# davidea97/Fisher-Nerf-customized

Hardware: AMD Instinct MI355X
Metric: candidate-views/sec (higher is better)
Workload: dtype f32

## Files before the change

### fisher-nerf-customized_amd/csrc/fisher_rast.hip

```cpp
#include <hip/hip_runtime.h>
#include <hip/hip_fp16.h>
#include <stdint.h>
#include <stdio.h>
#include <stdlib.h>
#include <string.h>
#include "fr_math.h"
#include "../../include/fisher_rast.h"
#include "fr_internal.h"

#define FR_THREADS 256
#define FR_G_MAX 32
#define FR_MAX_LDS_TILES 4096
#define FR_PART_MIN_DEFAULT 2048
#define FR_SORT_SMALL_KEYS 2048
#define FR_SORT_MID_KEYS 4096
#define FR_SORT_BIG_KEYS 16384
#define FR_VC_MAX 16
#define FR_BATCH 256
#define FR_BWD_BATCH 128

#include <vector>
#include <utility>
static thread_local char g_err[512] = "";
#if defined(FR_ABLATE) || defined(FR_LOOPSTATS)
#ifndef FR_AB
#define FR_AB
#endif
#endif
#ifdef FR_AB
#define FR_AB_ONLY(x) x
static int fr_debug_mode();
static int fr_env_int(const char* name) { const char* e = getenv(name); return e ? atoi(e) : 0; }
#else
#define FR_AB_ONLY(x)
static constexpr int fr_debug_mode() { return 0; }
#endif
static bool g_prof_on = false;
static std::vector<std::pair<hipEvent_t, hipEvent_t>> g_prof_events;
int fr_fail(int code, const char* msg)
{
	snprintf(g_err, sizeof(g_err), "%s", msg);
	return code;
}
int fr_check_launch(const char* what)
{
	hipError_t e = hipGetLastError();
	if (e != hipSuccess)
	{
		snprintf(g_err, sizeof(g_err), "%s: %s", what, hipGetErrorString(e));
		return FR_ELAUNCH;
	}
	return FR_OK;
}

struct FrSplat { float x, y, cx, cy, cz, o, depth; uint32_t ext; };

struct FrVisEntry { uint32_t idx, depth_bits, xy0, xy1; };

struct FrParams {
	int P, V, W, H;
	uint32_t gx, gy;
	int T;
	int G;
	float tanfovx, tanfovy, focal_x, focal_y, mod;
	int D, M;
	const float* bg; const float* view; const float* proj; const float* campos;
	const float* w2c;
	const float* means3D; const float* colors; const float* shs; const float* opac;
	const float* scales; const float* rots;
	const float* cov3D;
	float* cov3D_out;
	int* radii;
	FrSplat* splat;
	float* rgb;
	uint8_t* clamped;
	uint32_t* tile_cnt; uint32_t* tile_off; uint32_t* tile_fill;
	uint64_t* keys; long long key_capacity;
	uint32_t* blk_base;
	uint32_t* big_list;
	uint32_t* view_work;
	uint32_t* view_perm;
	int* status;
	int* vis_count;
	int* num_rendered;
	struct FrVisEntry* vis_list;
	uint32_t* vis_n;
	int VC;
	uint32_t tile_cap;
	uint32_t small_max;
	const uint32_t* order;
	int legacy_sort;
	int prefiltered;
	int ablate;
};
#ifdef FR_ABLATE
#define FR_ABL(x) x
#else
#define FR_ABL(x)
#endif

__device__ __forceinline__ float wave_sum(float v)
{
#pragma unroll
	for (int o = 32; o > 0; o >>= 1) v += __shfl_xor(v, o, 64);
	return v;
}
__device__ __forceinline__ int wave_max_i(int v)
{
#pragma unroll
	for (int o = 32; o > 0; o >>= 1) { int t = __shfl_xor(v, o, 64); v = t > v ? t : v; }
	return v;
}

__device__ __forceinline__ bool fr_any(bool x) { return __builtin_amdgcn_ballot_w64(x) != 0ull; }
__device__ __forceinline__ bool fr_all(bool x) { return __builtin_amdgcn_ballot_w64(!x) == 0ull; }
__device__ __forceinline__ float fr_readlane_f(float x, int l) { return __int_as_float(__builtin_amdgcn_readlane(__float_as_int(x), l)); }
__device__ __forceinline__ float fr_bperm_f(float x, int l) { return __int_as_float(__builtin_amdgcn_ds_bpermute(l << 2, __float_as_int(x))); }

__device__ __forceinline__ float fr_exp_hw(float x) { return __builtin_amdgcn_exp2f(x * 1.44269504088896341f); }

__device__ __forceinline__ float fr_power_threshold(float opacity)
{
	return (opacity > 0.f) ? (-__logf(255.0f * opacity) - 0.01f) : INFINITY;
}

__device__ __forceinline__ uint32_t fr_alpha_extent(float cx, float cy, float cz, float opacity)
{
	const float thr = fr_power_threshold(opacity);
	float hx = INFINITY, hy = INFINITY;
	if (!(thr <= 0.f)) { hx = -1.f; hy = -1.f; }
	else
	{
		const float det = cx * cz - cy * cy;
		if (det > 0.f && cx > 0.f && cz > 0.f)
		{
			const float tau2 = -2.0f * thr;
			const float ex = sqrtf(tau2 * cz / det) * 1.01f + 0.01f;
			const float ey = sqrtf(tau2 * cx / det) * 1.01f + 0.01f;
			if (ex == ex && ey == ey) { hx = ex; hy = ey; }
		}
	}
	const __half2 h = __halves2half2(__float2half_ru(hx), __float2half_ru(hy));
	return *(const uint32_t*)&h;
}

__global__ __launch_bounds__(FR_THREADS) void k_cov3d(int P, const float* __restrict__ scales, float mod,
                                                      const float* __restrict__ rots, float* __restrict__ cov3D)
{
	int i = blockIdx.x * FR_THREADS + threadIdx.x;
	if (i >= P) return;
	fr_f3 s = { scales[3 * i], scales[3 * i + 1], scales[3 * i + 2] };
	fr_f4 q = { rots[4 * i], rots[4 * i + 1], rots[4 * i + 2], rots[4 * i + 3] };
	float c[6];
	fr_cov3d(s, mod, q, c);
#pragma unroll
	for (int k = 0; k < 6; k++) cov3D[6 * (size_t)i + k] = c[k];
}

__global__ __launch_bounds__(FR_THREADS) void k_mark_visible(int P, const float* __restrict__ means3D,
                                                             const float* __restrict__ view, uint8_t* __restrict__ present)
{
	int i = blockIdx.x * FR_THREADS + threadIdx.x;
	if (i >= P) return;
	float vm[16];
#pragma unroll
	for (int k = 0; k < 16; k++) vm[k] = view[k];
	fr_f3 p = { means3D[3 * i], means3D[3 * i + 1], means3D[3 * i + 2] };
	fr_f3 pv = fr_xform4x3(p, vm);
	present[i] = (pv.z <= 0.001f) ? 0 : 1;
}

__global__ __launch_bounds__(FR_THREADS) void k_preprocess(FrParams p)
{
	extern __shared__ uint32_t fr_dyn_lds[];
// ... 1021 lines not shown
		{
			const int v = v0 + vv;
			uint32_t* cnt = p.tile_cnt + (size_t)v * p.T;
			const uint32_t* h = hist + (size_t)vv * p.T;
			for (int t = tid; t < p.T; t += FR_THREADS)
			{
				const uint32_t c = h[t];
				if (c) p.blk_base[((size_t)v * nblk + blockIdx.x) * p.T + t] = atomicAdd(&cnt[t], c);
			}
		}
	}
	if (tid < nv)
	{
		const int v = v0 + tid;
		p.vis_n[(size_t)v * nblk + blockIdx.x] = s_n[tid];
		if (p.vis_count && s_n[tid]) atomicAdd(&p.vis_count[v], (int)s_n[tid]);
		if (p.num_rendered && s_ref[tid]) atomicAdd(&p.num_rendered[v], (int)s_ref[tid]);
	}
}
__global__ __launch_bounds__(FR_THREADS) void k_scatter_vis(FrParams p)
{
	extern __shared__ uint32_t fr_dyn_lds[];
	uint32_t* s_cnt = fr_dyn_lds;
	uint32_t* s_base = fr_dyn_lds + p.T;
	if (p.status[1]) return;
	const int tid = threadIdx.x;
	const int v = blockIdx.y;
	const uint32_t nblk = gridDim.x;
	const uint32_t n = p.vis_n[(size_t)v * nblk + blockIdx.x];
	if (n == 0) return;
	const uint32_t* off = p.tile_off + (size_t)v * p.T;
	const uint32_t* bb = p.blk_base + ((size_t)v * nblk + blockIdx.x) * p.T;
	for (int t = tid; t < p.T; t += FR_THREADS) { s_cnt[t] = 0; s_base[t] = off[t] + bb[t]; }
	__syncthreads();
	const uint4* list = (const uint4*)(p.vis_list + ((size_t)v * nblk + blockIdx.x) * (size_t)(FR_THREADS * p.G));
	constexpr int NB = 4;
	for (uint32_t e0 = 0; e0 < n; e0 += NB * FR_THREADS)
	{
		uint4 en[NB];
#pragma unroll
		for (int b = 0; b < NB; b++)
		{
			const uint32_t e = e0 + b * FR_THREADS + tid;
			en[b] = e < n ? list[e] : make_uint4(0u, 0u, 0u, 0u);
		}
#pragma unroll
		for (int b = 0; b < NB; b++)
		{
			const uint64_t key = ((uint64_t)en[b].y << 32) | en[b].x;
			const uint32_t x0 = en[b].z & 0xffffu, y0 = en[b].z >> 16, x1 = en[b].w & 0xffffu, y1 = en[b].w >> 16;
			for (uint32_t y = y0; y < y1; y++)
				for (uint32_t x = x0; x < x1; x++)
				{
					const uint32_t t = y * p.gx + x;
					p.keys[s_base[t] + atomicAdd(&s_cnt[t], 1u)] = key;
				}
		}
	}
}

__device__ __forceinline__ void fr_tile_of_block(const FrParams& p, uint32_t& tile, int& v)
{
	const uint32_t L = blockIdx.x;
	if ((p.V & 7) == 0)
	{
		const uint32_t xcd = L & 7u, q = L >> 3;
		v = (int)((q / (uint32_t)p.T) * 8u + xcd);
		if (p.view_perm) v = (int)p.view_perm[v];
		tile = q % (uint32_t)p.T;
	}
	else
	{
		v = (int)(L / (uint32_t)p.T);
		tile = L % (uint32_t)p.T;
	}
}

__device__ __forceinline__ void fr_cx(uint64_t& lo, uint64_t& hi)
{
	const uint64_t a = lo, b = hi;
	const bool sw = a > b;
	lo = sw ? b : a; hi = sw ? a : b;
}
template <typename KeyPtr>
__device__ __forceinline__ uint64_t fr_ldk(KeyPtr keys, uint32_t i, uint32_t n) { return i < n ? keys[i] : ~0ull; }
template <typename KeyPtr>
__device__ __forceinline__ void fr_stk(KeyPtr keys, uint32_t i, uint32_t n, uint64_t v) { if (i < n) keys[i] = v; }

template <typename KeyPtr>
__device__ __forceinline__ void fr_bitonic(KeyPtr keys, uint32_t n, int tid, const uint32_t FR_NT = FR_THREADS)
{
	uint32_t n_pad = 1;
	while (n_pad < n) n_pad <<= 1;
	if (n_pad < 2) return;
	for (uint32_t t = tid; t < (n_pad >> 1); t += FR_NT)
	{
		uint64_t a = fr_ldk(keys, 2 * t, n), b = fr_ldk(keys, 2 * t + 1, n);
		fr_cx(a, b);
		fr_stk(keys, 2 * t, n, a); fr_stk(keys, 2 * t + 1, n, b);
	}
	__syncthreads();
	const uint32_t groups = n_pad >> 2;
	for (uint32_t k = 4, lk = 2; k <= n_pad; k <<= 1, lk++)
	{
		{
			const uint32_t q = k >> 2, qm = q - 1u;
			for (uint32_t g = tid; g < groups; g += FR_NT)
			{
				const uint32_t base = (g >> (lk - 2)) << lk, r = g & qm;
				const uint32_t ia = base + r, ib = ia + q, id = base + k - 1u - r, ic = id - q;
				uint64_t a = fr_ldk(keys, ia, n), b = fr_ldk(keys, ib, n), c = fr_ldk(keys, ic, n), d = fr_ldk(keys, id, n);
				fr_cx(a, d); fr_cx(b, c);
				fr_cx(a, b); fr_cx(c, d);
				fr_stk(keys, ia, n, a); fr_stk(keys, ib, n, b); fr_stk(keys, ic, n, c); fr_stk(keys, id, n, d);
			}
			__syncthreads();
		}
		uint32_t j = k >> 3, lj = lk - 3;
		for (; j >= 2; j >>= 2, lj -= 2)
		{
			const uint32_t h = j >> 1, lh = lj - 1, hm = h - 1u;
			for (uint32_t g = tid; g < groups; g += FR_NT)
			{
				const uint32_t i0 = ((g >> lh) << (lh + 2)) + (g & hm);
				const uint32_t i1 = i0 + h, i2 = i0 + j, i3 = i2 + h;
				uint64_t a = fr_ldk(keys, i0, n), b = fr_ldk(keys, i1, n), c = fr_ldk(keys, i2, n), d = fr_ldk(keys, i3, n);
				fr_cx(a, c); fr_cx(b, d);
				fr_cx(a, b); fr_cx(c, d);
				fr_stk(keys, i0, n, a); fr_stk(keys, i1, n, b); fr_stk(keys, i2, n, c); fr_stk(keys, i3, n, d);
			}
			__syncthreads();
		}
		if (j == 1)
		{
			for (uint32_t t = tid; t < (n_pad >> 1); t += FR_NT)
			{
				uint64_t a = fr_ldk(keys, 2 * t, n), b = fr_ldk(keys, 2 * t + 1, n);
				fr_cx(a, b);
				fr_stk(keys, 2 * t, n, a); fr_stk(keys, 2 * t + 1, n, b);
			}
			__syncthreads();
		}
	}
}

__device__ __forceinline__ uint64_t fr_shfl64(uint64_t v, int src_lane)
{
	const int lo = __builtin_amdgcn_ds_bpermute(src_lane << 2, (int)(uint32_t)v);
	const int hi = __builtin_amdgcn_ds_bpermute(src_lane << 2, (int)(uint32_t)(v >> 32));
	return ((uint64_t)(uint32_t)hi << 32) | (uint64_t)(uint32_t)lo;
}
__device__ __forceinline__ void fr_take(uint64_t& mine, uint64_t other, bool keepmin)
{
	const bool take = (other < mine) == keepmin;
	mine = take ? other : mine;
}
template <int CTRL>
__device__ __forceinline__ uint64_t fr_dpp64(uint64_t v)
{
	const int lo = __builtin_amdgcn_mov_dpp((int)(uint32_t)v, CTRL, 0xf, 0xf, false);
	const int hi = __builtin_amdgcn_mov_dpp((int)(uint32_t)(v >> 32), CTRL, 0xf, 0xf, false);
	return ((uint64_t)(uint32_t)hi << 32) | (uint64_t)(uint32_t)lo;
}
template <int ROWS>
__device__ __forceinline__ void fr_take_rows(uint64_t& key, bool keepmin)
{
	const uint32_t l = (uint32_t)key, h = (uint32_t)(key >> 32);
	uint64_t a, b;
	if constexpr (ROWS == 16)
	{
		const auto tl = __builtin_amdgcn_permlane16_swap(l, l, false, false);
		const auto th = __builtin_amdgcn_permlane16_swap(h, h, false, false);
		a = ((uint64_t)th[0] << 32) | tl[0]; b = ((uint64_t)th[1] << 32) | tl[1];
	}
	else
	{
		const auto tl = __builtin_amdgcn_permlane32_swap(l, l, false, false);
		const auto th = __builtin_amdgcn_permlane32_swap(h, h, false, false);
		a = ((uint64_t)th[0] << 32) | tl[0]; b = ((uint64_t)th[1] << 32) | tl[1];
	}
	key = ((b < a) == keepmin) ? b : a;
}

template <int K> struct FrLog2 { static constexpr int value = K == 1 ? 0 : K == 2 ? 1 : K == 4 ? 2 : K == 8 ? 3 : 4; };
template <int M>
__device__ __forceinline__ void fr_take_lane_xor(uint64_t& key, bool keepmin)
{
	if constexpr (M == 0) fr_take(key, fr_dpp64<0xB1>(key), keepmin);
	else if constexpr (M == 1) fr_take(key, fr_dpp64<0x4E>(key), keepmin);
	else if constexpr (M == 2) fr_take(key, fr_dpp64<0x141>(fr_dpp64<0x1B>(key)), keepmin);
	else if constexpr (M == 3) fr_take(key, fr_dpp64<0x128>(key), keepmin);
	else if constexpr (M == 4) fr_take_rows<16>(key, keepmin);
	else fr_take_rows<32>(key, keepmin);
}
template <int M>
__device__ __forceinline__ uint64_t fr_lane_mirror(uint64_t key, int lane)
{
	if constexpr (M == 1) return fr_dpp64<0xB1>(key);
	else if constexpr (M == 2) return fr_dpp64<0x1B>(key);
	else if constexpr (M == 3) return fr_dpp64<0x141>(key);
	else if constexpr (M == 4) return fr_dpp64<0x140>(key);
	else return fr_shfl64(key, lane ^ ((1 << M) - 1));
}

template <int K, int S>
__device__ __forceinline__ void fr_wave_flip(uint64_t (&key)[K], int lane)
{
	constexpr int LK = FrLog2<K>::value;
	if constexpr (S <= LK)
	{
		constexpr int kr = 1 << S;
#pragma unroll
		for (int r = 0; r < K; r++)
			if ((r & (kr >> 1)) == 0) fr_cx(key[r], key[r ^ (kr - 1)]);
	}
	else
	{
		constexpr int M = S - LK;
		const bool keepmin = (lane & (1 << (M - 1))) == 0;
		if constexpr (K == 1) fr_take(key[0], fr_lane_mirror<M>(key[0], lane), keepmin);
		else
		{
#pragma unroll
			for (int r = 0; r < K / 2; r++)
			{
				const uint64_t lo = key[r], hi = key[K - 1 - r];
				fr_take(key[r], fr_lane_mirror<M>(hi, lane), keepmin);
				fr_take(key[K - 1 - r], fr_lane_mirror<M>(lo, lane), keepmin);
			}
		}
	}
}
template <int K, int T>
__device__ __forceinline__ void fr_wave_xor_down(uint64_t (&key)[K], int lane)
{
	constexpr int LK = FrLog2<K>::value;
	if constexpr (T >= 0)
	{
		if constexpr (T >= LK)
		{
			const bool keepmin = (lane & (1 << (T - LK))) == 0;
#pragma unroll
			for (int r = 0; r < K; r++) fr_take_lane_xor<T - LK>(key[r], keepmin);
		}
		else
		{
			constexpr int jr = 1 << T;
#pragma unroll
			for (int r = 0; r < K; r++)
				if ((r & jr) == 0) fr_cx(key[r], key[r | jr]);
		}
		fr_wave_xor_down<K, T - 1>(key, lane);
	}
}
template <int K, int S>
__device__ __forceinline__ void fr_wave_stages(uint64_t (&key)[K], uint32_t n_pad, int lane)
{
	if constexpr (S >= 1)
	{
		fr_wave_stages<K, S - 1>(key, n_pad, lane);
		if ((1u << S) <= n_pad)
		{
			fr_wave_flip<K, S>(key, lane);
			fr_wave_xor_down<K, S - 2>(key, lane);
		}
	}
}

template <int K>
__device__ __forceinline__ void fr_sort_wave_segment(uint64_t* __restrict__ gk, uint32_t n, int lane)
{
	uint64_t key[K];
#pragma unroll
	for (int r = 0; r < K; r++) { const uint32_t i = (uint32_t)(lane * K + r); key[r] = i < n ? gk[i] : ~0ull; }
	uint32_t n_pad = 1;
	while (n_pad < n) n_pad <<= 1;
	fr_wave_stages<K, 6 + FrLog2<K>::value>(key, n_pad, lane);
#pragma unroll
	for (int r = 0; r < K; r++) { const uint32_t i = (uint32_t)(lane * K + r); if (i < n) gk[i] = key[r]; }
}

template <int K, int NW, int TW>
__device__ __forceinline__ void fr_wg_xor_down(uint64_t (&key)[K], uint64_t* sk, int w, int lane)
{
	if constexpr (TW >= 0)
	{
		constexpr int RUN = 64 * K, jw = 1 << TW;
		const uint32_t base = (uint32_t)(w * RUN);
#pragma unroll
		for (int r = 0; r < K; r++) sk[base + (uint32_t)(r * 64 + lane)] = key[r];
		__syncthreads();
		const uint32_t pbase = (uint32_t)((w ^ jw) * RUN);
		const bool keepmin = (w & jw) == 0;
#pragma unroll
		for (int r = 0; r < K; r++) fr_take(key[r], sk[pbase + (uint32_t)(r * 64 + lane)], keepmin);
		__syncthreads();
		fr_wg_xor_down<K, NW, TW - 1>(key, sk, w, lane);
	}
}
template <int K, int NW, int SW>
__device__ __forceinline__ void fr_wg_stages(uint64_t (&key)[K], uint64_t* sk, uint32_t n_pad, int w, int lane)
{
	if constexpr (SW >= 1)
	{
		fr_wg_stages<K, NW, SW - 1>(key, sk, n_pad, w, lane);
		constexpr int RUN = 64 * K, kw = 1 << SW;
		if (((uint32_t)RUN << SW) <= n_pad)
		{
			const uint32_t base = (uint32_t)(w * RUN);
#pragma unroll
			for (int r = 0; r < K; r++) sk[base + (uint32_t)(r * 64 + lane)] = key[r];
			__syncthreads();
			const uint32_t pbase = (uint32_t)((w ^ (kw - 1)) * RUN);
			const bool keepmin = (w & (kw >> 1)) == 0;
#pragma unroll
			for (int r = 0; r < K; r++) fr_take(key[r], sk[pbase + (uint32_t)((K - 1 - r) * 64 + (63 - lane))], keepmin);
			__syncthreads();
			fr_wg_xor_down<K, NW, SW - 2>(key, sk, w, lane);
			fr_wave_xor_down<K, 5 + FrLog2<K>::value>(key, lane);
		}
	}
}

template <int K, int NW>
__device__ __forceinline__ void fr_sort_wg_segment(uint64_t* sk, uint64_t* __restrict__ gk, uint32_t n, int tid)
{
	static_assert(NW == 4 || NW == 16, "4 or 16 waves");
	constexpr int RUN = 64 * K;
	const int lane = tid & 63;
	const int w = __builtin_amdgcn_readfirstlane(tid >> 6);
	const uint32_t base = (uint32_t)(w * RUN);
	uint64_t key[K];
#pragma unroll
	for (int r = 0; r < K; r++) { const uint32_t i = base + (uint32_t)(lane * K + r); key[r] = i < n ? gk[i] : ~0ull; }
	uint32_t n_pad = 1;
	while (n_pad < n) n_pad <<= 1;
	fr_wave_stages<K, 6 + FrLog2<K>::value>(key, n_pad, lane);
	fr_wg_stages<K, NW, (NW == 4 ? 2 : 4)>(key, sk, n_pad, w, lane);
#pragma unroll
	for (int r = 0; r < K; r++) { const uint32_t i = base + (uint32_t)(lane * K + r); if (i < n) gk[i] = key[r]; }
}

__global__ __launch_bounds__(FR_THREADS) void k_sort_tiles(FrParams p)
{
	if (p.status[1]) return;
	__shared__ uint64_t skeys[FR_SORT_SMALL_KEYS];
	const int tid = threadIdx.x;
	uint32_t tile; int v;
	fr_tile_of_block(p, tile, v);
	const size_t vt = (size_t)v * p.T + tile;
	const uint32_t n = p.tile_cnt[vt];
	if (n < 2 || n > p.small_max) return;
	uint64_t* gk = p.keys + p.tile_off[vt];
#ifdef FR_AB
	if (p.legacy_sort)
	{
		for (uint32_t i = tid; i < n; i += FR_THREADS) skeys[i] = gk[i];
		__syncthreads();
		fr_bitonic(skeys, n, tid, FR_THREADS);
		for (uint32_t i = tid; i < n; i += FR_THREADS) gk[i] = skeys[i];
		return;
	}
#endif
	if (n <= 512u)
	{
		if (tid >= 64) return;
		if (n <= 64u) fr_sort_wave_segment<1>(gk, n, tid);
		else if (n <= 128u) fr_sort_wave_segment<2>(gk, n, tid);
		else if (n <= 256u) fr_sort_wave_segment<4>(gk, n, tid);
		else fr_sort_wave_segment<8>(gk, n, tid);
		return;
	}
	if (n <= 1024u) fr_sort_wg_segment<4, 4>(skeys, gk, n, tid);
	else fr_sort_wg_segment<8, 4>(skeys, gk, n, tid);
}

#define FR_PART_SAMPLE 512
#define FR_PART_MAXP 64
__global__ __launch_bounds__(FR_THREADS) void k_sort_part(FrParams p, uint32_t part_max)
{
	__shared__ uint64_t skeys[FR_SORT_SMALL_KEYS];
	__shared__ uint64_t s_piv[FR_PART_MAXP];
	__shared__ uint32_t s_cnt[FR_PART_MAXP], s_off[FR_PART_MAXP], s_cur[FR_PART_MAXP];
	__shared__ uint32_t s_next;
	if (p.status[1]) return;
	const int tid = threadIdx.x, lane = tid & 63;
	const uint32_t count = p.big_list[0];
	for (uint32_t b = blockIdx.x; b < count; b += gridDim.x)
	{
		const size_t vt = p.big_list[16 + b];
		const uint32_t n = p.tile_cnt[vt];
		if (n > part_max) continue;
		uint64_t* gk = p.keys + p.tile_off[vt];
		const uint32_t n_al = (n + 63u) & ~63u;
		uint64_t* tmp = gk + n_al;
		const uint32_t NP = n <= 1280u ? 4u : n <= 2560u ? 8u : n <= 5120u ? 16u : n <= 10240u ? 32u : 64u;
		__syncthreads();
		if (tid < FR_PART_MAXP) { s_cnt[tid] = 0u; s_cur[tid] = 0u; }
		if (tid == 0) s_next = 0u;
		if (tid < 64)
		{
			uint64_t key[8];
#pragma unroll
			for (int r = 0; r < 8; r++) key[r] = gk[(uint32_t)(((uint64_t)(uint32_t)(lane * 8 + r) * n) >> 9)];
			fr_wave_stages<8, 9>(key, (uint32_t)FR_PART_SAMPLE, lane);
			const uint32_t step = 64u / NP;
			if (((uint32_t)lane % step) == 0u && lane > 0) s_piv[(uint32_t)lane / step] = key[0];
		}
		__syncthreads();
		auto part_of = [&](uint64_t k) -> uint32_t {
			uint32_t lo = 0u;
			for (uint32_t stepw = NP >> 1; stepw > 0u; stepw >>= 1)
			{
				const uint32_t mid = lo + stepw;
				if (s_piv[mid] <= k) lo = mid;
			}
			return lo;
		};
		constexpr int KB = 8;
		for (uint32_t i0 = 0; i0 < n; i0 += KB * FR_THREADS)
		{
			uint64_t k[KB];
#pragma unroll
			for (int r = 0; r < KB; r++) { const uint32_t i = i0 + r * FR_THREADS + tid; k[r] = i < n ? gk[i] : ~0ull; }
#pragma unroll
			for (int r = 0; r < KB; r++) { const uint32_t i = i0 + r * FR_THREADS + tid; if (i < n) atomicAdd(&s_cnt[part_of(k[r])], 1u); }
		}
		__syncthreads();
		if (tid == 0)
		{
			uint32_t run = 0;
			for (uint32_t q = 0; q < NP; q++) { s_off[q] = run; run += s_cnt[q]; }
		}
		__syncthreads();
		for (uint32_t i0 = 0; i0 < n; i0 += KB * FR_THREADS)
		{
			uint64_t k[KB];
#pragma unroll
			for (int r = 0; r < KB; r++) { const uint32_t i = i0 + r * FR_THREADS + tid; k[r] = i < n ? gk[i] : ~0ull; }
#pragma unroll
			for (int r = 0; r < KB; r++)
			{
				const uint32_t i = i0 + r * FR_THREADS + tid;
				if (i < n) { const uint32_t q = part_of(k[r]); tmp[s_off[q] + atomicAdd(&s_cur[q], 1u)] = k[r]; }
			}
		}
		__syncthreads();
		for (;;)
		{
			uint32_t q = 0;
			if (lane == 0) q = atomicAdd(&s_next, 1u);
			q = (uint32_t)__builtin_amdgcn_readfirstlane((int)q);
			if (q >= NP) break;
			const uint32_t c = s_cnt[q];
			uint64_t* pk = tmp + s_off[q];
			if (c < 2u || c > 512u) continue;
			if (c <= 64u) fr_sort_wave_segment<1>(pk, c, lane);
			else if (c <= 128u) fr_sort_wave_segment<2>(pk, c, lane);
			else if (c <= 256u) fr_sort_wave_segment<4>(pk, c, lane);
			else fr_sort_wave_segment<8>(pk, c, lane);
		}
		__syncthreads();
		for (uint32_t q = 0; q < NP; q++)
		{
			const uint32_t c = s_cnt[q];
			if (c <= 512u) continue;
			uint64_t* pk = tmp + s_off[q];
			if (c <= 1024u) fr_sort_wg_segment<4, 4>(skeys, pk, c, tid);
			else if (c <= (uint32_t)FR_SORT_SMALL_KEYS) fr_sort_wg_segment<8, 4>(skeys, pk, c, tid);
			else fr_bitonic(pk, c, tid, FR_THREADS);
			__syncthreads();
		}
		if (tid == 0) p.tile_off[vt] += n_al;
	}
}

__global__ __launch_bounds__(FR_THREADS) void k_sort_mid_tiles(FrParams p, uint32_t part_max)
{
	if (p.status[1]) return;
	__shared__ uint64_t skeys[FR_SORT_MID_KEYS];
	const int tid = threadIdx.x;
	const uint32_t count = p.big_list[0];
	for (uint32_t b = blockIdx.x; b < count; b += gridDim.x)
	{
		const size_t vt = p.big_list[16 + b];
		const uint32_t n = p.tile_cnt[vt];
		if (n > (uint32_t)FR_SORT_MID_KEYS || n <= part_max) continue;
		uint64_t* gk = p.keys + p.tile_off[vt];
		__syncthreads();
#ifdef FR_AB
		if (p.legacy_sort)
		{
			for (uint32_t i = tid; i < n; i += FR_THREADS) skeys[i] = gk[i];
			__syncthreads();
			fr_bitonic(skeys, n, tid, FR_THREADS);
			for (uint32_t i = tid; i < n; i += FR_THREADS) gk[i] = skeys[i];
		}
		else
#endif
		fr_sort_wg_segment<16, 4>(skeys, gk, n, tid);
	}
}

__global__ __launch_bounds__(1024) void k_sort_big_tiles(FrParams p, uint32_t part_max)
{
	if (p.status[1]) return;
	__shared__ uint64_t skeys[FR_SORT_BIG_KEYS];
	const int tid = threadIdx.x;
	const uint32_t count = p.big_list[0];
	for (uint32_t b = blockIdx.x; b < count; b += gridDim.x)
	{
		const size_t vt = p.big_list[16 + b];
		const uint32_t n = p.tile_cnt[vt];
		if (n <= (uint32_t)FR_SORT_MID_KEYS || n <= part_max) continue;
		uint64_t* gk = p.keys + p.tile_off[vt];
		__syncthreads();
		if (n > (uint32_t)FR_SORT_BIG_KEYS) fr_bitonic(gk, n, tid, 1024);
#ifdef FR_AB
		else if (p.legacy_sort)
		{
			for (uint32_t i = tid; i < n; i += 1024) skeys[i] = gk[i];
			__syncthreads();
			fr_bitonic(skeys, n, tid, 1024);
			for (uint32_t i = tid; i < n; i += 1024) gk[i] = skeys[i];
		}
#endif
		else if (n <= 8192u) fr_sort_wg_segment<8, 16>(skeys, gk, n, tid);
		else fr_sort_wg_segment<16, 16>(skeys, gk, n, tid);
	}
}

__device__ __forceinline__ bool fr_pair_alpha(float xyx, float xyy, float pfx, float pfy, float cx, float cy, float cz,
                                              float o, float thr, float& dx, float& dy, float& G, float& alpha)
{
	dx = xyx - pfx; dy = xyy - pfy;
	const float power = -0.5f * (cx * dx * dx + cz * dy * dy) - cy * dx * dy;
	if (power > 0.0f) return false;
	if (power < thr) return false;
	G = fr_expf(power);
	alpha = fminf(0.99f, o * G);
	if (alpha < 1.0f / 255.0f) return false;
	return true;
}

template <int NCH>
__global__ __launch_bounds__(FR_THREADS) void k_render_forward(FrParams p, const float* __restrict__ feat, int feat_view_stride,
                                                               float* __restrict__ final_T, uint32_t* __restrict__ n_contrib,
                                                               float* __restrict__ out_color, float* __restrict__ out_depth,
                                                               const float* __restrict__ feat2, float* __restrict__ out_color2)
{
	if (p.status[1]) return;
	const int tid = threadIdx.x, lane = tid & 63;
// ... 4210 lines not shown
	L.final_T = o; o = fr_align(o + (size_t)(V * W * H) * 4);
	L.n_contrib = o; o = fr_align(o + (size_t)(V * W * H) * 4);
	L.status = o; o = fr_align(o + 64);
	L.big_list = o; o = fr_align(o + (size_t)(V * T) * 4 + 64);
	L.blk_base = o; o = fr_align(o + (T <= FR_MAX_LDS_TILES ? (size_t)V * (size_t)fr_preprocess_blocks(P, V) * (size_t)T * 4 : 0));
	L.img_bytes = o;
	L.keys = 0;
	L.bin_bytes = fr_align((size_t)(max_rendered > 0 ? max_rendered : 1) * 8);
	return L;
}

extern "C" int fr_version(void) { return FR_VERSION; }
#ifndef FR_SRC_HASH
#define FR_SRC_HASH "unstamped"
#endif
extern "C" const char* fr_build_id(void) { return FR_SRC_HASH; }
extern "C" const char* fr_last_error(void) { return g_err; }

extern "C" int fr_workspace_bytes(int32_t P, int32_t W, int32_t H, int64_t max_rendered, size_t out[3])
{
	if (P < 0 || W <= 0 || H <= 0 || max_rendered < 0 || !out) return fr_fail(FR_EINVAL, "fr_workspace_bytes: bad argument");
	FrLayout L = fr_layout(P, W, H, 1, max_rendered);
	out[0] = L.geom_bytes; out[1] = L.bin_bytes; out[2] = L.img_bytes;
	return FR_OK;
}

extern "C" int fr_workspace_layout(int32_t P, int32_t W, int32_t H, int64_t max_rendered, size_t o[11])
{
	if (P < 0 || W <= 0 || H <= 0 || max_rendered < 0 || !o) return fr_fail(FR_EINVAL, "fr_workspace_layout: bad argument");
	FrLayout L = fr_layout(P, W, H, 1, max_rendered);
	o[0] = L.splat; o[1] = L.cov3D; o[2] = L.rgb; o[3] = L.clamped;
	o[4] = L.tile_cnt; o[5] = L.tile_off; o[6] = L.tile_fill; o[7] = L.final_T; o[8] = L.n_contrib; o[9] = L.status;
	o[10] = L.keys;
	return FR_OK;
}

extern "C" int fr_mark_visible(int32_t P, const float* means3D, const float* viewmatrix, const float* projmatrix,
                               uint8_t* present, fr_stream_t stream)
{
	(void)projmatrix;
	if (P < 0) return fr_fail(FR_EINVAL, "fr_mark_visible: P < 0");
	if (P == 0) return FR_OK;
	if (!means3D || !viewmatrix || !present) return fr_fail(FR_EINVAL, "fr_mark_visible: null pointer");
	hipLaunchKernelGGL(k_mark_visible, dim3((P + FR_THREADS - 1) / FR_THREADS), dim3(FR_THREADS), 0, (hipStream_t)stream,
	                   P, means3D, viewmatrix, present);
	return fr_check_launch("k_mark_visible");
}

static int fr_validate(const fr_raster_cfg* cfg, const fr_gaussians* g, const char* who, bool need_opacity = true)
{
	static thread_local char buf[256];
	if (!cfg || !g) { snprintf(buf, sizeof(buf), "%s: null cfg/gaussians", who); return fr_fail(FR_EINVAL, buf); }
	if (cfg->P < 0 || cfg->image_width <= 0 || cfg->image_height <= 0) { snprintf(buf, sizeof(buf), "%s: bad P/W/H", who); return fr_fail(FR_EINVAL, buf); }
	if (cfg->P == 0) return FR_OK;
	if (!g->means3D || (need_opacity && !g->opacities) || !cfg->bg || !cfg->viewmatrix || !cfg->projmatrix)
	{ snprintf(buf, sizeof(buf), "%s: null means3D/opacities/bg/viewmatrix/projmatrix", who); return fr_fail(FR_EINVAL, buf); }
	if ((g->colors_precomp == nullptr) == (g->shs == nullptr))
	{ snprintf(buf, sizeof(buf), "%s: provide exactly one of SHs or precomputed colors", who); return fr_fail(FR_EINVAL, buf); }
	if (g->shs && (!cfg->campos || cfg->sh_coeffs <= 0 || (cfg->sh_degree + 1) * (cfg->sh_degree + 1) > cfg->sh_coeffs || cfg->sh_degree > 3 || cfg->sh_degree < 0))
	{ snprintf(buf, sizeof(buf), "%s: bad SH degree / coefficient count / campos", who); return fr_fail(FR_EINVAL, buf); }
	const bool sr = g->scales && g->rotations;
	if ((sr ? 1 : 0) + (g->cov3D_precomp ? 1 : 0) != 1 || ((g->scales != nullptr) != (g->rotations != nullptr)))
	{ snprintf(buf, sizeof(buf), "%s: provide exactly one of scale/rotation pair or precomputed 3D covariance", who); return fr_fail(FR_EINVAL, buf); }
	return FR_OK;
}

static void fr_fill_params(FrParams& p, const fr_raster_cfg* cfg, const fr_gaussians* g, int V)
{
	memset(&p, 0, sizeof(p));
	p.P = cfg->P; p.V = V; p.W = cfg->image_width; p.H = cfg->image_height;
	p.gx = (uint32_t)((p.W + 15) / 16); p.gy = (uint32_t)((p.H + 15) / 16); p.T = (int)(p.gx * p.gy);
	p.tanfovx = cfg->tanfovx; p.tanfovy = cfg->tanfovy;
	p.focal_y = p.H / (2.0f * cfg->tanfovy);
	p.focal_x = p.W / (2.0f * cfg->tanfovx);
	p.mod = cfg->scale_modifier; p.D = cfg->sh_degree; p.M = cfg->sh_coeffs;
	p.prefiltered = cfg->prefiltered;
	p.bg = cfg->bg; p.view = cfg->viewmatrix; p.proj = cfg->projmatrix; p.campos = cfg->campos;
	p.means3D = g->means3D; p.colors = g->colors_precomp; p.shs = g->shs; p.opac = g->opacities;
	p.scales = g->scales; p.rots = g->rotations;
	p.VC = 1;
	p.small_max = FR_SORT_SMALL_KEYS;
	p.order = nullptr;
	p.legacy_sort = fr_debug_mode() == 6;
	FR_ABL(p.ablate = fr_debug_mode();)
}

#define FR_ZERO_MAX 12
struct FrZeroList { uint32_t* ptr[FR_ZERO_MAX]; unsigned long long end[FR_ZERO_MAX]; unsigned long long dwords[FR_ZERO_MAX]; int n; };
__global__ __launch_bounds__(FR_THREADS) void k_zero_many(FrZeroList z)
{
	const unsigned long long total = z.end[z.n - 1];
	for (unsigned long long i = (unsigned long long)blockIdx.x * FR_THREADS + threadIdx.x; i < total; i += (unsigned long long)gridDim.x * FR_THREADS)
	{
		int b = 0;
		while (i >= z.end[b]) b++;
		const unsigned long long u = i - (b ? z.end[b - 1] : 0ull);
		uint32_t* q = z.ptr[b] + 4 * u;
		if (4 * u + 4 <= z.dwords[b] && ((uintptr_t)q & 15u) == 0) *(uint4*)q = make_uint4(0u, 0u, 0u, 0u);
		else
			for (unsigned long long k = 4 * u; k < 4 * u + 4 && k < z.dwords[b]; k++) z.ptr[b][k] = 0u;
	}
}
struct FrZeroer {
	FrZeroList z; unsigned long long run = 0;
	FrZeroer() { z.n = 0; }
	void add(void* p, size_t bytes) { if (!p || bytes == 0) return; z.ptr[z.n] = (uint32_t*)p; z.dwords[z.n] = bytes / 4; run += (bytes / 4 + 3) / 4; z.end[z.n] = run; z.n++; }
	void launch(hipStream_t s)
	{
		if (z.n == 0) return;
		const unsigned long long blocks = (run + FR_THREADS * 4 - 1) / (FR_THREADS * 4);
		hipLaunchKernelGGL(k_zero_many, dim3((unsigned)(blocks > 4096 ? 4096 : (blocks < 1 ? 1 : blocks))), dim3(FR_THREADS), 0, s, z);
	}
};

struct FrSideStream {
	hipStream_t stream = nullptr; hipEvent_t fork = nullptr, join = nullptr; bool ok = false; int device = -1;
};
static FrSideStream& fr_side_stream(int which = 0)
{
	static thread_local FrSideStream sides[3];
	FrSideStream& ss = sides[which];
	int dev = -1;
	(void)hipGetDevice(&dev);
	if (ss.device != dev)
	{
		if (ss.ok) { (void)hipEventDestroy(ss.fork); (void)hipEventDestroy(ss.join); (void)hipStreamDestroy(ss.stream); }
#ifdef FR_AB
		static const int tile_prio = fr_env_int("FR_TILE_PRIO");
#else
		constexpr int tile_prio = 0;
#endif
		int lo = 0, hi = 0;
		(void)hipDeviceGetStreamPriorityRange(&lo, &hi);
		const int prio = (which == 2 && tile_prio > 0) ? lo : (which == 2 && tile_prio < 0) ? hi : 0;
		ss.ok = hipStreamCreateWithPriority(&ss.stream, hipStreamNonBlocking, prio) == hipSuccess
		     && hipEventCreateWithFlags(&ss.fork, hipEventDisableTiming) == hipSuccess
		     && hipEventCreateWithFlags(&ss.join, hipEventDisableTiming) == hipSuccess;
		ss.device = dev;
		(void)hipGetLastError();
	}
	return ss;
}

struct FrJoinGuard {
	hipStream_t s; FrSideStream* side[2] = { nullptr, nullptr }; int n = 0;
	explicit FrJoinGuard(hipStream_t caller) : s(caller) {}
	void forked(FrSideStream* ss) { side[n++] = ss; }
	int join()
	{
		int rc = FR_OK;
		for (int i = 0; i < n; i++)
		{
			if (hipEventRecord(side[i]->join, side[i]->stream) != hipSuccess || hipStreamWaitEvent(s, side[i]->join, 0) != hipSuccess)
				rc = fr_fail(FR_ELAUNCH, "side stream join failed");
		}
		n = 0;
		return rc;
	}
	~FrJoinGuard() { if (n) { char keep[sizeof(g_err)]; memcpy(keep, g_err, sizeof(keep)); (void)join(); memcpy(g_err, keep, sizeof(keep)); } }
};

struct FrScorerPlan { int columns; bool form_a; FrRecordArgs ra; bool skip_pack = false; bool general = false; bool pose = false; };
template <int C> __global__ void k_pack_static(FrParams p, const float* __restrict__ H_inv, float* __restrict__ packed, float4* __restrict__ mt, float4* __restrict__ grp);
template <int C, bool LIST, bool FORM_A> __global__ void k_fisher_records(FrParams p, FrRecordArgs ra);

static int fr_bin_pipeline(FrParams& p, const fr_gaussians* g, hipStream_t s, const FrScorerPlan* plan = nullptr)
// ... 1476 lines not shown
```

Before: 45100.

## Sort tile keys via 32-bit depth surrogates with fixup and fallback

```diff
diff --git a/fisher-nerf-customized_amd/csrc/fisher_rast.hip b/fisher-nerf-customized_amd/csrc/fisher_rast.hip
--- a/fisher-nerf-customized_amd/csrc/fisher_rast.hip
+++ b/fisher-nerf-customized_amd/csrc/fisher_rast.hip
@@ -90,6 +90,7 @@
 	uint32_t small_max;
 	const uint32_t* order;
 	int legacy_sort;
+	int sort64;
 	int prefiltered;
 	int ablate;
 };
@@ -1277,6 +1278,11 @@
 	const bool sw = a > b;
 	lo = sw ? b : a; hi = sw ? a : b;
 }
+__device__ __forceinline__ void fr_cx(uint32_t& lo, uint32_t& hi)
+{
+	const uint32_t a = lo, b = hi;
+	lo = min(a, b); hi = max(a, b);
+}
 template <typename KeyPtr>
 __device__ __forceinline__ uint64_t fr_ldk(KeyPtr keys, uint32_t i, uint32_t n) { return i < n ? keys[i] : ~0ull; }
 template <typename KeyPtr>
@@ -1345,7 +1351,11 @@
 	const int hi = __builtin_amdgcn_ds_bpermute(src_lane << 2, (int)(uint32_t)(v >> 32));
 	return ((uint64_t)(uint32_t)hi << 32) | (uint64_t)(uint32_t)lo;
 }
-__device__ __forceinline__ void fr_take(uint64_t& mine, uint64_t other, bool keepmin)
+__device__ __forceinline__ uint32_t fr_shfl32(uint32_t v, int src_lane) { return (uint32_t)__builtin_amdgcn_ds_bpermute(src_lane << 2, (int)v); }
+__device__ __forceinline__ uint64_t fr_shflk(uint64_t v, int src_lane) { return fr_shfl64(v, src_lane); }
+__device__ __forceinline__ uint32_t fr_shflk(uint32_t v, int src_lane) { return fr_shfl32(v, src_lane); }
+template <typename Key>
+__device__ __forceinline__ void fr_take(Key& mine, Key other, bool keepmin)
 {
 	const bool take = (other < mine) == keepmin;
 	mine = take ? other : mine;
@@ -1357,6 +1367,8 @@
 	const int hi = __builtin_amdgcn_mov_dpp((int)(uint32_t)(v >> 32), CTRL, 0xf, 0xf, false);
 	return ((uint64_t)(uint32_t)hi << 32) | (uint64_t)(uint32_t)lo;
 }
+template <int CTRL> __device__ __forceinline__ uint64_t fr_dppk(uint64_t v) { return fr_dpp64<CTRL>(v); }
+template <int CTRL> __device__ __forceinline__ uint32_t fr_dppk(uint32_t v) { return (uint32_t)__builtin_amdgcn_mov_dpp((int)v, CTRL, 0xf, 0xf, false); }
 template <int ROWS>
 __device__ __forceinline__ void fr_take_rows(uint64_t& key, bool keepmin)
 {
@@ -1376,30 +1388,38 @@
 	}
 	key = ((b < a) == keepmin) ? b : a;
 }
+template <int ROWS>
+__device__ __forceinline__ void fr_take_rows(uint32_t& key, bool keepmin)
+{
+	uint32_t a, b;
+	if constexpr (ROWS == 16) { const auto t = __builtin_amdgcn_permlane16_swap(key, key, false, false); a = t[0]; b = t[1]; }
+	else { const auto t = __builtin_amdgcn_permlane32_swap(key, key, false, false); a = t[0]; b = t[1]; }
+	key = keepmin ? min(a, b) : max(a, b);
+}
 
 template <int K> struct FrLog2 { static constexpr int value = K == 1 ? 0 : K == 2 ? 1 : K == 4 ? 2 : K == 8 ? 3 : 4; };
-template <int M>
-__device__ __forceinline__ void fr_take_lane_xor(uint64_t& key, bool keepmin)
-{
-	if constexpr (M == 0) fr_take(key, fr_dpp64<0xB1>(key), keepmin);
-	else if constexpr (M == 1) fr_take(key, fr_dpp64<0x4E>(key), keepmin);
-	else if constexpr (M == 2) fr_take(key, fr_dpp64<0x141>(fr_dpp64<0x1B>(key)), keepmin);
-	else if constexpr (M == 3) fr_take(key, fr_dpp64<0x128>(key), keepmin);
+template <int M, typename Key>
+__device__ __forceinline__ void fr_take_lane_xor(Key& key, bool keepmin)
+{
+	if constexpr (M == 0) fr_take(key, fr_dppk<0xB1>(key), keepmin);
+	else if constexpr (M == 1) fr_take(key, fr_dppk<0x4E>(key), keepmin);
+	else if constexpr (M == 2) fr_take(key, fr_dppk<0x141>(fr_dppk<0x1B>(key)), keepmin);
+	else if constexpr (M == 3) fr_take(key, fr_dppk<0x128>(key), keepmin);
 	else if constexpr (M == 4) fr_take_rows<16>(key, keepmin);
 	else fr_take_rows<32>(key, keepmin);
 }
-template <int M>
-__device__ __forceinline__ uint64_t fr_lane_mirror(uint64_t key, int lane)
-{
-	if constexpr (M == 1) return fr_dpp64<0xB1>(key);
-	else if constexpr (M == 2) return fr_dpp64<0x1B>(key);
-	else if constexpr (M == 3) return fr_dpp64<0x141>(key);
-	else if constexpr (M == 4) return fr_dpp64<0x140>(key);
-	else return fr_shfl64(key, lane ^ ((1 << M) - 1));
-}
-
-template <int K, int S>
-__device__ __forceinline__ void fr_wave_flip(uint64_t (&key)[K], int lane)
+template <int M, typename Key>
+__device__ __forceinline__ Key fr_lane_mirror(Key key, int lane)
+{
+	if constexpr (M == 1) return fr_dppk<0xB1>(key);
+	else if constexpr (M == 2) return fr_dppk<0x1B>(key);
+	else if constexpr (M == 3) return fr_dppk<0x141>(key);
+	else if constexpr (M == 4) return fr_dppk<0x140>(key);
+	else return fr_shflk(key, lane ^ ((1 << M) - 1));
+}
+
+template <int K, int S, typename Key>
+__device__ __forceinline__ void fr_wave_flip(Key (&key)[K], int lane)
 {
 	constexpr int LK = FrLog2<K>::value;
 	if constexpr (S <= LK)
@@ -1419,15 +1439,15 @@
 #pragma unroll
 			for (int r = 0; r < K / 2; r++)
 			{
-				const uint64_t lo = key[r], hi = key[K - 1 - r];
+				const Key lo = key[r], hi = key[K - 1 - r];
 				fr_take(key[r], fr_lane_mirror<M>(hi, lane), keepmin);
 				fr_take(key[K - 1 - r], fr_lane_mirror<M>(lo, lane), keepmin);
 			}
 		}
 	}
 }
-template <int K, int T>
-__device__ __forceinline__ void fr_wave_xor_down(uint64_t (&key)[K], int lane)
+template <int K, int T, typename Key>
+__device__ __forceinline__ void fr_wave_xor_down(Key (&key)[K], int lane)
 {
 	constexpr int LK = FrLog2<K>::value;
 	if constexpr (T >= 0)
@@ -1448,8 +1468,8 @@
 		fr_wave_xor_down<K, T - 1>(key, lane);
 	}
 }
-template <int K, int S>
-__device__ __forceinline__ void fr_wave_stages(uint64_t (&key)[K], uint32_t n_pad, int lane)
+template <int K, int S, typename Key>
+__device__ __forceinline__ void fr_wave_stages(Key (&key)[K], uint32_t n_pad, int lane)
 {
 	if constexpr (S >= 1)
 	{
@@ -1475,8 +1495,8 @@
 	for (int r = 0; r < K; r++) { const uint32_t i = (uint32_t)(lane * K + r); if (i < n) gk[i] = key[r]; }
 }
 
-template <int K, int NW, int TW>
-__device__ __forceinline__ void fr_wg_xor_down(uint64_t (&key)[K], uint64_t* sk, int w, int lane)
+template <int K, int NW, int TW, typename Key>
+__device__ __forceinline__ void fr_wg_xor_down(Key (&key)[K], Key* sk, int w, int lane)
 {
 	if constexpr (TW >= 0)
 	{
@@ -1493,8 +1513,8 @@
 		fr_wg_xor_down<K, NW, TW - 1>(key, sk, w, lane);
 	}
 }
-template <int K, int NW, int SW>
-__device__ __forceinline__ void fr_wg_stages(uint64_t (&key)[K], uint64_t* sk, uint32_t n_pad, int w, int lane)
+template <int K, int NW, int SW, typename Key>
+__device__ __forceinline__ void fr_wg_stages(Key (&key)[K], Key* sk, uint32_t n_pad, int w, int lane)
 {
 	if constexpr (SW >= 1)
 	{
@@ -1532,6 +1552,164 @@
 	while (n_pad < n) n_pad <<= 1;
 	fr_wave_stages<K, 6 + FrLog2<K>::value>(key, n_pad, lane);
 	fr_wg_stages<K, NW, (NW == 4 ? 2 : 4)>(key, sk, n_pad, w, lane);
+#pragma unroll
+	for (int r = 0; r < K; r++) { const uint32_t i = base + (uint32_t)(lane * K + r); if (i < n) gk[i] = key[r]; }
+}
+
+__device__ __forceinline__ uint32_t fr_wave_umin(uint32_t x)
+{
+#pragma unroll
+	for (int m = 1; m < 64; m <<= 1) x = min(x, fr_shfl32(x, (int)(__lane_id() ^ (uint32_t)m)));
+	return x;
+}
+__device__ __forceinline__ uint32_t fr_wave_umax(uint32_t x)
+{
+#pragma unroll
+	for (int m = 1; m < 64; m <<= 1) x = max(x, fr_shfl32(x, (int)(__lane_id() ^ (uint32_t)m)));
+	return x;
+}
+__device__ __forceinline__ uint32_t fr_sur_shift(uint32_t dmin, uint32_t dmax, uint32_t L)
+{
+	const uint32_t range = dmax - dmin;
+	const uint32_t bl = range ? 32u - (uint32_t)__builtin_clz(range) : 0u;
+	return bl > 32u - L ? bl - (32u - L) : 0u;
+}
+template <int K>
+__device__ __forceinline__ bool fr_wave_out_of_order(const uint64_t (&key)[K], int lane)
+{
+	bool bad = false;
+#pragma unroll
+	for (int r = 0; r + 1 < K; r++) bad |= key[r] > key[r + 1];
+	const uint64_t nxt = fr_shfl64(key[0], (lane + 1) & 63);
+	bad |= lane < 63 && key[K - 1] > nxt;
+	return bad;
+}
+#define FR_SUR_FIXUP 4
+template <int K>
+__device__ __forceinline__ bool fr_wave_fixup(uint64_t (&key)[K], int lane)
+{
+	bool bad = fr_any(fr_wave_out_of_order(key, lane));
+	for (int round = 0; bad && round < FR_SUR_FIXUP; round++)
+	{
+#pragma unroll
+		for (int r = 0; r + 1 < K; r += 2) fr_cx(key[r], key[r + 1]);
+#pragma unroll
+		for (int r = 1; r + 1 < K; r += 2) fr_cx(key[r], key[r + 1]);
+		const uint64_t nxt = fr_shfl64(key[0], (lane + 1) & 63), prv = fr_shfl64(key[K - 1], (lane - 1) & 63);
+		if (lane < 63 && nxt < key[K - 1]) key[K - 1] = nxt;
+		if (lane > 0 && prv > key[0]) key[0] = prv;
+		bad = fr_any(fr_wave_out_of_order(key, lane));
+	}
+	return bad;
+}
+
+template <int K>
+__device__ __forceinline__ void fr_wave_sort_sur(uint64_t (&key)[K], uint64_t* stage, uint32_t n, uint32_t n_pad, int lane)
+{
+	uint32_t dmin = ~0u, dmax = 0u;
+#pragma unroll
+	for (int r = 0; r < K; r++)
+	{
+		const uint32_t i = (uint32_t)(lane * K + r);
+		if (i < n)
+		{
+			stage[i] = key[r];
+			const uint32_t hi = (uint32_t)(key[r] >> 32);
+			dmin = min(dmin, hi); dmax = max(dmax, hi);
+		}
+	}
+	dmin = fr_wave_umin(dmin); dmax = fr_wave_umax(dmax);
+	const uint32_t L = (uint32_t)__builtin_ctz(n_pad), s = fr_sur_shift(dmin, dmax, L);
+	uint32_t sur[K];
+#pragma unroll
+	for (int r = 0; r < K; r++)
+	{
+		const uint32_t i = (uint32_t)(lane * K + r);
+		sur[r] = i < n ? ((((uint32_t)(key[r] >> 32) - dmin) >> s) << L) | i : ~0u;
+	}
+	fr_wave_stages<K, 6 + FrLog2<K>::value>(sur, n_pad, lane);
+	__builtin_amdgcn_wave_barrier();
+#pragma unroll
+	for (int r = 0; r < K; r++)
+	{
+		const uint32_t e = (uint32_t)(lane * K + r);
+		key[r] = e < n ? stage[sur[r] & (n_pad - 1u)] : ~0ull;
+	}
+	if (fr_wave_fixup(key, lane))
+	{
+#pragma unroll
+		for (int r = 0; r < K; r++) { const uint32_t i = (uint32_t)(lane * K + r); key[r] = i < n ? stage[i] : ~0ull; }
+		fr_wave_stages<K, 6 + FrLog2<K>::value>(key, n_pad, lane);
+	}
+}
+template <int K>
+__device__ __forceinline__ void fr_sort_wave_segment_sur(uint64_t* __restrict__ gk, uint64_t* stage, uint32_t n, int lane)
+{
+	uint64_t key[K];
+#pragma unroll
+	for (int r = 0; r < K; r++) { const uint32_t i = (uint32_t)(lane * K + r); key[r] = i < n ? gk[i] : ~0ull; }
+	uint32_t n_pad = 1;
+	while (n_pad < n) n_pad <<= 1;
+	fr_wave_sort_sur(key, stage, n, n_pad, lane);
+#pragma unroll
+	for (int r = 0; r < K; r++) { const uint32_t i = (uint32_t)(lane * K + r); if (i < n) gk[i] = key[r]; }
+}
+
+template <int K, int NW>
+__device__ __forceinline__ void fr_sort_wg_segment_sur(uint64_t* sk, uint64_t* __restrict__ gk, uint32_t n, int tid)
+{
+	static_assert(NW == 4 || NW == 16, "4 or 16 waves");
+	constexpr int RUN = 64 * K;
+	const int lane = tid & 63;
+	const int w = __builtin_amdgcn_readfirstlane(tid >> 6);
+	const uint32_t base = (uint32_t)(w * RUN);
+	uint64_t key[K];
+	uint32_t dmin = ~0u, dmax = 0u;
+#pragma unroll
+	for (int r = 0; r < K; r++)
+	{
+		const uint32_t i = base + (uint32_t)(lane * K + r);
+		key[r] = i < n ? gk[i] : ~0ull;
+		if (i < n) { const uint32_t hi = (uint32_t)(key[r] >> 32); dmin = min(dmin, hi); dmax = max(dmax, hi); }
+	}
+	uint32_t* s32 = reinterpret_cast<uint32_t*>(sk);
+	dmin = fr_wave_umin(dmin); dmax = fr_wave_umax(dmax);
+	if (lane == 0) { s32[2 * w] = dmin; s32[2 * w + 1] = dmax; }
+	__syncthreads();
+#pragma unroll
+	for (int x = 0; x < NW; x++) { dmin = min(dmin, s32[2 * x]); dmax = max(dmax, s32[2 * x + 1]); }
+	__syncthreads();
+	uint32_t n_pad = 1;
+	while (n_pad < n) n_pad <<= 1;
+	const uint32_t L = (uint32_t)__builtin_ctz(n_pad), s = fr_sur_shift(dmin, dmax, L);
+	uint32_t sur[K];
+#pragma unroll
+	for (int r = 0; r < K; r++)
+	{
+		const uint32_t i = base + (uint32_t)(lane * K + r);
+		sur[r] = i < n ? ((((uint32_t)(key[r] >> 32) - dmin) >> s) << L) | i : ~0u;
+	}
+	fr_wave_stages<K, 6 + FrLog2<K>::value>(sur, n_pad, lane);
+	fr_wg_stages<K, NW, (NW == 4 ? 2 : 4)>(sur, s32, n_pad, w, lane);
+#pragma unroll
+	for (int r = 0; r < K; r++)
+	{
+		const uint32_t e = base + (uint32_t)(lane * K + r);
+		key[r] = e < n ? gk[sur[r] & (n_pad - 1u)] : ~0ull;
+	}
+	bool bad = fr_wave_fixup(key, lane);
+	if (lane == 0) sk[w] = key[0];
+	if (tid == 0) s32[2 * NW] = 0u;
+	__syncthreads();
+	if (lane == 63 && w + 1 < NW) bad |= key[K - 1] > sk[w + 1];
+	if (bad) s32[2 * NW] = 1u;
+	__syncthreads();
+	if (s32[2 * NW])
+	{
+		__syncthreads();
+		fr_sort_wg_segment<K, NW>(sk, gk, n, tid);
+		return;
+	}
 #pragma unroll
 	for (int r = 0; r < K; r++) { const uint32_t i = base + (uint32_t)(lane * K + r); if (i < n) gk[i] = key[r]; }
 }
@@ -1557,17 +1735,33 @@
 		return;
 	}
 #endif
+#ifdef FR_AB
+	if (p.sort64)
+	{
+		if (n <= 512u)
+		{
+			if (tid >= 64) return;
+			if (n <= 64u) fr_sort_wave_segment<1>(gk, n, tid);
+			else if (n <= 128u) fr_sort_wave_segment<2>(gk, n, tid);
+			else if (n <= 256u) fr_sort_wave_segment<4>(gk, n, tid);
+			else fr_sort_wave_segment<8>(gk, n, tid);
+		}
+		else if (n <= 1024u) fr_sort_wg_segment<4, 4>(skeys, gk, n, tid);
+		else fr_sort_wg_segment<8, 4>(skeys, gk, n, tid);
+		return;
+	}
+#endif
 	if (n <= 512u)
 	{
 		if (tid >= 64) return;
 		if (n <= 64u) fr_sort_wave_segment<1>(gk, n, tid);
-		else if (n <= 128u) fr_sort_wave_segment<2>(gk, n, tid);
-		else if (n <= 256u) fr_sort_wave_segment<4>(gk, n, tid);
-		else fr_sort_wave_segment<8>(gk, n, tid);
+		else if (n <= 128u) fr_sort_wave_segment_sur<2>(gk, skeys, n, tid);
+		else if (n <= 256u) fr_sort_wave_segment_sur<4>(gk, skeys, n, tid);
+		else fr_sort_wave_segment_sur<8>(gk, skeys, n, tid);
 		return;
 	}
-	if (n <= 1024u) fr_sort_wg_segment<4, 4>(skeys, gk, n, tid);
-	else fr_sort_wg_segment<8, 4>(skeys, gk, n, tid);
+	if (n <= 1024u) fr_sort_wg_segment_sur<4, 4>(skeys, gk, n, tid);
+	else fr_sort_wg_segment_sur<8, 4>(skeys, gk, n, tid);
 }
 
 #define FR_PART_SAMPLE 512
@@ -1598,7 +1792,8 @@
 			uint64_t key[8];
 #pragma unroll
 			for (int r = 0; r < 8; r++) key[r] = gk[(uint32_t)(((uint64_t)(uint32_t)(lane * 8 + r) * n) >> 9)];
-			fr_wave_stages<8, 9>(key, (uint32_t)FR_PART_SAMPLE, lane);
+			if (FR_AB_ONLY(p.sort64 ||) false) fr_wave_stages<8, 9>(key, (uint32_t)FR_PART_SAMPLE, lane);
+			else fr_wave_sort_sur(key, skeys, (uint32_t)FR_PART_SAMPLE, (uint32_t)FR_PART_SAMPLE, lane);
 			const uint32_t step = 64u / NP;
 			if (((uint32_t)lane % step) == 0u && lane > 0) s_piv[(uint32_t)lane / step] = key[0];
 		}
@@ -1650,10 +1845,17 @@
 			const uint32_t c = s_cnt[q];
 			uint64_t* pk = tmp + s_off[q];
 			if (c < 2u || c > 512u) continue;
-			if (c <= 64u) fr_sort_wave_segment<1>(pk, c, lane);
-			else if (c <= 128u) fr_sort_wave_segment<2>(pk, c, lane);
-			else if (c <= 256u) fr_sort_wave_segment<4>(pk, c, lane);
-			else fr_sort_wave_segment<8>(pk, c, lane);
+			uint64_t* stage = skeys + (tid >> 6) * 512;
+			if (c <= 64u || FR_AB_ONLY(p.sort64 ||) false)
+			{
+				if (c <= 64u) fr_sort_wave_segment<1>(pk, c, lane);
+				else if (c <= 128u) fr_sort_wave_segment<2>(pk, c, lane);
+				else if (c <= 256u) fr_sort_wave_segment<4>(pk, c, lane);
+				else fr_sort_wave_segment<8>(pk, c, lane);
+			}
+			else if (c <= 128u) fr_sort_wave_segment_sur<2>(pk, stage, c, lane);
+			else if (c <= 256u) fr_sort_wave_segment_sur<4>(pk, stage, c, lane);
+			else fr_sort_wave_segment_sur<8>(pk, stage, c, lane);
 		}
 		__syncthreads();
 		for (uint32_t q = 0; q < NP; q++)
@@ -1661,8 +1863,8 @@
 			const uint32_t c = s_cnt[q];
 			if (c <= 512u) continue;
 			uint64_t* pk = tmp + s_off[q];
-			if (c <= 1024u) fr_sort_wg_segment<4, 4>(skeys, pk, c, tid);
-			else if (c <= (uint32_t)FR_SORT_SMALL_KEYS) fr_sort_wg_segment<8, 4>(skeys, pk, c, tid);
+			if (c <= 1024u) fr_sort_wg_segment_sur<4, 4>(skeys, pk, c, tid);
+			else if (c <= (uint32_t)FR_SORT_SMALL_KEYS) fr_sort_wg_segment_sur<8, 4>(skeys, pk, c, tid);
 			else fr_bitonic(pk, c, tid, FR_THREADS);
 			__syncthreads();
 		}
@@ -6039,6 +6241,7 @@
 	p.small_max = FR_SORT_SMALL_KEYS;
 	p.order = nullptr;
 	p.legacy_sort = fr_debug_mode() == 6;
+	p.sort64 = fr_debug_mode() == 38;
 	FR_ABL(p.ablate = fr_debug_mode();)
 }
 
```

After: 45710, median of 6. 1.01x the previous value.
